# BayesLIM/BayesLIM

Hardware: AMD Instinct MI355X
Metric: visibilities/sec (Nbl x Ntime x Nfreq) fwd+bwd (higher is better)
Workload: dtype f32 (fringe sum: f16x3 split operands on the f16 MFMA -- 22-bit operands, f32 accumulate; phases f64); 1 GPU; HERA-128 (8128 bl), nside=128 diffuse + 1e4 point sources, 256 freqs; Nbl=8128, Nfreqs=256, Npix_sky=182664, Npix_visible=98304, Npoint=10000, beam=Airy D=14m on 1deg rect grid, linear PixelBeam interp, loss=sum |V|^2 (fused chi-square epilogue, rime_chisq_fwd / _bwd), parallelism=channel-sharded x1

## Files before the change

### bayeslim_amd/csrc/fringe_mfma.hip

```cpp
#include <hip/hip_runtime.h>
#include <hip/hip_fp16.h>
#include <type_traits>
#include "rime_common.h"

namespace rime {

typedef float f32x16 __attribute__((ext_vector_type(16)));
typedef _Float16 f16x8 __attribute__((ext_vector_type(8)));
typedef _Float16 f16x2 __attribute__((ext_vector_type(2)));

constexpr int MF_NA = 128;
constexpr int MF_SPLIT_PIX = 16384;

struct AntArgs {
    const double* antpos;
    const double* sdir;
    const double* freqs;
    const float* psky;
    const float* scale;
    const float* rowmin;
    const int* pair_direct;
    const int* pair_conj;
    float* vis;
    float* ws;
// ... 862 lines not shown
                if constexpr (!CEN) {
                    split2(w0 * c0, w1 * c1, rh, rl);
                    split2(w0 * s0, w1 * s1, ih, il);
                } else {
                    float xr0, xr1, xi0, xi1;
                    split2_prod(w0, c0, w1, c1, xr0, xr1, rh, rl);
                    split2_prod(w0, s0, w1, s1, xi0, xi1, ih, il);
                    cr[u] = fmaf(g0, xr0, cr[u]); keep_scalar(cr[u]); ci[u] = fmaf(g0, xi0, ci[u]);
                    cr[u] = fmaf(g1, xr1, cr[u]); keep_scalar(cr[u]); ci[u] = fmaf(g1, xi1, ci[u]);
                }
                unsigned char* o = buf + octet_row(u) * MF_ROWB + pp * 4 + 32 * hf;
                *reinterpret_cast<uint32_t*>(o) = rh;
                *reinterpret_cast<uint32_t*>(o + 2 * MF_KP) = ih;
                *reinterpret_cast<uint32_t*>(o + MF_IMG) = rl;
                *reinterpret_cast<uint32_t*>(o + MF_IMG + 2 * MF_KP) = il;
            }
        }
        fetch(next_panel);
    };

    const int foff = (lane & 31) * MF_ROWB + (lane >> 5) * 16;
    auto contract = [&](const unsigned char* buf) {
        auto frag = [&](int tile, int img, int im, int ks) {
            return *reinterpret_cast<const uint4*>(buf + img * MF_IMG + tile * 32 * MF_ROWB + foff + im * 2 * MF_KP + 32 * ks);
        };
        auto sgn = [&](uint4 v, const uint4& sg) {
            if constexpr (SIGNED) { v.x ^= sg.x; v.y ^= sg.y; v.z ^= sg.z; v.w ^= sg.w; }
            return v;
        };
#pragma unroll
        for (int ks = 0; ks < MF_NH; ++ks) {
            uint4 sg = make_uint4(0, 0, 0, 0);
            if constexpr (SIGNED) sg = *reinterpret_cast<const uint4*>(buf + 2 * MF_IMG + (2 * ks + (lane >> 5)) * 16);
            if constexpr (W == 0) {
                const uint4 Lrh = sgn(frag(0, 0, 0, ks), sg), Lih = sgn(frag(0, 0, 1, ks), sg);
                const uint4 Lrl = sgn(frag(0, 1, 0, ks), sg), Lil = sgn(frag(0, 1, 1, ks), sg);
                const uint4 Brh = frag(1, 0, 0, ks), Bih = frag(1, 0, 1, ks), Brl = frag(1, 1, 0, ks), Bil = frag(1, 1, 1, ks);
                acc[0] = RIME_MFMA(Lrh, Brh, acc[0]);
                acc[1] = RIME_MFMA(Lih, Bih, acc[1]);
                acc[0] = RIME_MFMA(Lrh, Brl, acc[0]);
                acc[1] = RIME_MFMA(Lih, Bil, acc[1]);
                acc[0] = RIME_MFMA(Lrl, Brh, acc[0]);
                acc[1] = RIME_MFMA(Lil, Bih, acc[1]);
            } else if constexpr (W == 1) {
                const uint4 Lrh = sgn(frag(0, 0, 0, ks), sg), Lih = sgn(frag(0, 0, 1, ks), sg);
                const uint4 Lrl = sgn(frag(0, 1, 0, ks), sg), Lil = sgn(frag(0, 1, 1, ks), sg);
                const uint4 Brh = frag(1, 0, 0, ks), Bih = frag(1, 0, 1, ks), Brl = frag(1, 1, 0, ks), Bil = frag(1, 1, 1, ks);
                acc[0] = RIME_MFMA(Lrh, Bih, acc[0]);
                acc[1] = RIME_MFMA(Lih, Brh, acc[1]);
                acc[0] = RIME_MFMA(Lrh, Bil, acc[0]);
                acc[1] = RIME_MFMA(Lih, Brl, acc[1]);
                acc[0] = RIME_MFMA(Lrl, Bih, acc[0]);
                acc[1] = RIME_MFMA(Lil, Brh, acc[1]);
            } else {
                constexpr int tt = W - 2;
                const uint4 Brh = frag(tt, 0, 0, ks), Bih = frag(tt, 0, 1, ks), Brl = frag(tt, 1, 0, ks), Bil = frag(tt, 1, 1, ks);
                const uint4 Lrh = sgn(Brh, sg), Lih = sgn(Bih, sg);
                const uint4 Hr = half_frag(Lrh), Hi = half_frag(Lih);
                acc[0] = RIME_MFMA(Hr, Brh, acc[0]);
                acc[1] = RIME_MFMA(Hi, Bih, acc[1]);
                acc[2] = RIME_MFMA(Lrh, Bih, acc[2]);
                acc[0] = RIME_MFMA(Lrh, Brl, acc[0]);
                acc[1] = RIME_MFMA(Lih, Bil, acc[1]);
                acc[3] = RIME_MFMA(Lih, Brl, acc[3]);
                acc[2] = RIME_MFMA(Lrh, Bil, acc[2]);
            }
        }
    };

    unsigned char* const buf0 = smem;
    unsigned char* const buf1 = smem + MF_BUF;
    fetch(pbeg);
    generate(buf0, min(pbeg + 1, pend - 1));
    __syncthreads();
    for (int panel = pbeg; panel < pend; panel += 2) {
        if (panel + 1 < pend) generate(buf1, min(panel + 2, pend - 1));
        contract(buf0);
        __syncthreads();
        if (panel + 1 < pend) {
            if (panel + 2 < pend) generate(buf0, min(panel + 3, pend - 1));
            contract(buf1);
        }
        __syncthreads();
    }

    float* dst = A.ws + (((size_t)split * A.Nt + t) * A.Nf + f) * 2 * A.Nbl;
    const float inv = 1.0f / scl;
    const int col = lane & 31, rb = 4 * (lane >> 5);
    RIME_MFMA_SETTLE();
    auto put = [&](int r, int c, float vr, float vi) {
        const int bd = A.pair_direct[r * MF_NA + c];
        if (bd >= 0) { dst[bd] = vr; dst[(size_t)A.Nbl + bd] = vi; }
        const int bc = A.pair_conj[r * MF_NA + c];
        if (bc >= 0) { dst[bc] = vr; dst[(size_t)A.Nbl + bc] = -vi; }
    };
    auto put1 = [&](int r, int c, int im, float v) {
        const int bd = A.pair_direct[r * MF_NA + c];
        if (bd >= 0) dst[(size_t)im * A.Nbl + bd] = v;
        const int bc = A.pair_conj[r * MF_NA + c];
        if (bc >= 0) dst[(size_t)im * A.Nbl + bc] = im ? -v : v;
    };
    if constexpr (CEN) {
#pragma unroll
        for (int u = 0; u < NGEN; ++u)
#pragma unroll
            for (int o = 1; o < 8; o <<= 1) { cr[u] += __shfl_xor(cr[u], o, 64); keep_scalar(cr[u]); ci[u] += __shfl_xor(ci[u], o, 64); keep_scalar(ci[u]); }
        float* cs = reinterpret_cast<float*>(smem) + 4 * (32 * 33);
        if (pp == 0) {
#pragma unroll
            for (int u = 0; u < NGEN; ++u)
                if (u < nk) { cs[(hf * 64 + octet_row(u)) * 2] = cr[u]; cs[(hf * 64 + octet_row(u)) * 2 + 1] = ci[u]; }
        }
        __syncthreads();
        if (tid < A.Nant) {
            float vr = cs[tid * 2] + cs[(64 + tid) * 2], vi = cs[tid * 2 + 1] + cs[(64 + tid) * 2 + 1];
            keep_scalar(vr); keep_scalar(vi);
            vr *= inv; keep_scalar(vr); vi *= inv;
            int b = A.centre[tid];
            if (b >= 0) { dst[b] = vr; dst[(size_t)A.Nbl + b] = vi; }
            b = A.centre[MF_NA + tid];
            if (b >= 0) { dst[b] = vr; dst[(size_t)A.Nbl + b] = -vi; }
            b = A.centre[64 + tid];
            if (b >= 0) { dst[b] = vr; dst[(size_t)A.Nbl + b] = -vi; }
            b = A.centre[MF_NA + 64 + tid];
            if (b >= 0) { dst[b] = vr; dst[(size_t)A.Nbl + b] = vi; }
        }
    }
    float* tr = reinterpret_cast<float*>(smem) + W * (32 * 33);
    auto transposed = [&](const f32x16& v) {
        f32x16 tv;
#pragma unroll
        for (int e = 0; e < 16; ++e) tr[((e & 3) + 8 * (e >> 2) + rb) * 33 + col] = v[e];
        asm volatile("s_waitcnt lgkmcnt(0)" ::: "memory");
#pragma unroll
        for (int e = 0; e < 16; ++e) tv[e] = tr[col * 33 + (e & 3) + 8 * (e >> 2) + rb];
        asm volatile("s_waitcnt lgkmcnt(0)" ::: "memory");
        return tv;
    };
    if constexpr (W < 2) {
        f32x16 s, d;
#pragma unroll
        for (int e = 0; e < 16; ++e) { s[e] = (acc[0][e] + acc[1][e]) * inv; d[e] = (acc[0][e] - acc[1][e]) * inv; }
        const f32x16 st = transposed(s), dt = transposed(d);
#pragma unroll
        for (int e = 0; e < 16; ++e) {
            const int re = (e & 3) + 8 * (e >> 2) + rb;
            const int i = re, j = 32 + col;
            const int it = col, jt = 32 + re;
            if constexpr (W == 0) {
                put1(i, j, 0, s[e]); put1(i, 64 + j, 0, d[e]);
                put1(64 + it, 64 + jt, 0, st[e]); put1(jt, 64 + it, 0, dt[e]);
            } else {
                put1(i, j, 1, d[e]); put1(i, 64 + j, 1, -s[e]);
                put1(64 + it, 64 + jt, 1, -dt[e]); put1(jt, 64 + it, 1, -st[e]);
            }
        }
    } else {
        constexpr int tt = W - 2;
        f32x16 ar, br, ai, bi, x, y;
#pragma unroll
        for (int e = 0; e < 16; ++e) { x[e] = acc[0][e] + acc[1][e]; y[e] = acc[0][e] - acc[1][e]; }
// ... 590 lines not shown
#pragma unroll
            for (int e = 0; e < 16; ++e) {
                const int an = 32 * ti + (e & 3) + 8 * (e >> 2) + 4 * h;
                const double ph = phase3(ant_lds[3 * an], sx, ant_lds[3 * an + 1], sy, ant_lds[3 * an + 2], sz);
                const float rr = turn_frac(ph);
                const float ce = __builtin_amdgcn_cosf(rr), se = __builtin_amdgcn_sinf(rr);
                part = fmaf(ce, accR[ti][e], part);
                part = fmaf(se, accI[ti][e], part);
                if constexpr (CPLX) {
                    pa = fmaf(se, accR[ti][e], pa);
                    pb = fmaf(ce, accI[ti][e], pb);
                }
                if ((e & 3) == 3) __builtin_amdgcn_sched_barrier(0);
            }
            if constexpr (CPLX) parti += pa - pb;
        }
        part += __shfl_xor(part, 32, 64);
        if constexpr (CPLX) parti += __shfl_xor(parti, 32, 64);
        if (h == 0) {
            float* o = orow + (size_t)p * A.st_p;
            if constexpr (CPLX) {
                const float im = parti * inv * A.imsign;
                float2* o2 = reinterpret_cast<float2*>(o);
                *o2 = A.accumulate ? make_float2(o2->x + part * inv, o2->y + im) : make_float2(part * inv, im);
            } else {
                *o = A.accumulate ? *o + part * inv : part * inv;
            }
        }
    }
}

struct PairBwdArgs : AntBwdArgs {
    const int* centre;
};

template <int TF> constexpr int pb_plane() { return (TF == 1 ? 1 : 3) * 2 * 2 * 32 * 16; }
constexpr int PB_THREADS = 256;
template <int TF> constexpr size_t pb_lds() { return 8 * (size_t)pb_plane<TF>() + 64 * 3 * sizeof(double) + 2 * 64 * sizeof(float); }

template <bool CEN, bool FLAT, int TF>
__global__ void __launch_bounds__(PB_THREADS, 3)
fringe_pair_bwd_kernel(PairBwdArgs A)
{
    constexpr int PB_PLANE = pb_plane<TF>();
    extern __shared__ __align__(16) unsigned char smem[];
    unsigned char* g_img = smem;
    double* ant_lds = reinterpret_cast<double*>(smem + 8 * PB_PLANE);
    float* cen_u = reinterpret_cast<float*>(smem + 8 * PB_PLANE + 64 * 3 * sizeof(double));
    float* cen_v = cen_u + 64;

    const int tid = threadIdx.x, lane = tid & 63, wave = __builtin_amdgcn_readfirstlane(tid >> 6);
    const int f = blockIdx.x % A.Nf, ts = blockIdx.x / A.Nf;
    const int t = ts / A.S, split = ts % A.S;
    const int TA = (A.Nant + 31) / 32;

    const double nu_c = A.sign * A.freqs[f] * (1.0 / 2.99792458e8);
    for (int i = tid; i < 64 * 3; i += PB_THREADS) ant_lds[i] = (i < A.Nant * 3) ? nu_c * A.antpos[i] : 0.0;
    const float gs = A.gscale[t * A.Nf + f] * 0.125f;
    const float* gre = A.gvt + ((size_t)t * A.Nf + f) * 2 * A.Nbl;
    const float* gim = gre + A.Nbl;
    auto grad_of = [&](int r, int c, float& vr, float& vi) {
        const int bd = A.pair_direct[r * MF_NA + c];
        if (bd >= 0) { vr += gre[bd]; keep_scalar(vr); vi += gim[bd]; keep_scalar(vi); }
        const int bc = A.pair_conj[r * MF_NA + c];
        if (bc >= 0) { vr += gre[bc]; keep_scalar(vr); vi -= gim[bc]; keep_scalar(vi); }
    };
    auto entry = [&](int i, int j, bool off, float& ar, float& ai, float& br, float& bi) {
        float xr = 0.f, xi = 0.f, yr = 0.f, yi = 0.f;
        grad_of(i, j, xr, xi);
        grad_of(64 + i, 64 + j, yr, yi);
        ar = xr + yr; keep_scalar(ar); ai = yi - xi;
        br = 0.f; bi = 0.f;
        grad_of(j, 64 + i, br, bi);
        if (off) grad_of(i, 64 + j, br, bi);
    };
    for (int e = tid; e < (TF == 1 ? 1 : 3) * 2 * 2 * 32 * 4; e += PB_THREADS) {
        const int jp = e & 3, row = (e >> 2) & 31, h = (e >> 7) & 1, ks = (e >> 8) & 1, tile = e >> 9;
        const int ti = tile == 2 ? 1 : 0, tj = tile == 0 ? 0 : 1;
        const int i = 32 * ti + row;
        const int j0 = 32 * tj + ((2 * jp) & 3) + 8 * (2 * ks + (jp >> 1)) + 4 * h;
        float n1[2] = {0.f, 0.f}, n2[2] = {0.f, 0.f}, n3[2] = {0.f, 0.f}, n4[2] = {0.f, 0.f};
        if (tj < TA) {
#pragma unroll
            for (int q = 0; q < 2; ++q) {
                const int j = j0 + q;
                float ar, ai, br, bi;
                entry(i, j, ti != tj, ar, ai, br, bi);
                if (ti != tj) {
                    n1[q] = ar + br; keep_scalar(n1[q]); n2[q] = ar - br; keep_scalar(n2[q]);
                    n3[q] = -(ai + bi); keep_scalar(n3[q]); n4[q] = ai - bi;
// ... 32 lines not shown
            b = A.centre[64 + tid];
            if (b >= 0) { u += gre[b]; keep_scalar(u); v -= gim[b]; keep_scalar(v); }
            b = A.centre[MF_NA + 64 + tid];
            if (b >= 0) { u += gre[b]; keep_scalar(u); v += gim[b]; keep_scalar(v); }
            u *= gs; keep_scalar(u); v *= gs;
            cen_u[tid] = u; cen_v[tid] = v;
        }
    }
    __syncthreads();

    const double* sd = A.sdir + (size_t)t * 3 * A.Pstride;
    float* orow = A.gpsky + (size_t)t * A.st_t + (size_t)f * A.st_f;
    const float inv = 1.0f / gs;
    const int h = lane >> 5;
    const int ntile = A.Pstride / 32;
    const int tbeg = split * A.tiles_per_split;
    const int tend = min(ntile, tbeg + A.tiles_per_split);

    const uint32_t gl0 = (h * 32 + (lane & 31)) * 16;
    for (int pt = tbeg + wave; pt < tend; pt += PB_THREADS / 64) {
        const int p = pt * 32 + (lane & 31);
        const double sx = sd[p], sy = sd[A.Pstride + p], sz = FLAT ? 0.0 : sd[2 * (size_t)A.Pstride + p];
        f32x16 accR[TF], accI[TF];
#pragma unroll
        for (int q = 0; q < TF; ++q)
#pragma unroll
            for (int e = 0; e < 16; ++e) {
                if constexpr (CEN) {
                    accR[q][e] = cen_u[32 * q + (e & 3) + 8 * (e >> 2) + 4 * h];
                    accI[q][e] = cen_v[32 * q + (e & 3) + 8 * (e >> 2) + 4 * h];
                } else { accR[q][e] = 0.f; accI[q][e] = 0.f; }
            }
        float part = 0.f;
#pragma unroll
        for (int tjr = 0; tjr < TF; ++tjr) {
            const int tj = TF - 1 - tjr;
            if (tj < TA) {
                float ec[16], es[16];
#pragma unroll
                for (int ks = 0; ks < 2; ++ks) {
                    if (32 * tj + 16 * ks >= A.Nant) {
#pragma unroll
                        for (int jj = 0; jj < 8; ++jj) { ec[8 * ks + jj] = 0.f; es[8 * ks + jj] = 0.f; }
                        continue;
                    }
                    uint4 Erh, Erl, Eih, Eil;
                    uint32_t* erh = reinterpret_cast<uint32_t*>(&Erh); uint32_t* erl = reinterpret_cast<uint32_t*>(&Erl);
                    uint32_t* eih = reinterpret_cast<uint32_t*>(&Eih); uint32_t* eil = reinterpret_cast<uint32_t*>(&Eil);
#pragma unroll
                    for (int jq = 0; jq < 2; ++jq) {
                        if (32 * tj + 16 * ks + 8 * jq >= A.Nant) {
#pragma unroll
                            for (int u = 0; u < 4; ++u) { ec[8 * ks + 4 * jq + u] = 0.f; es[8 * ks + 4 * jq + u] = 0.f; }
                            continue;
                        }
#pragma unroll
                        for (int u = 0; u < 4; ++u) {
                            const int jj = 4 * jq + u;
                            const int an = 32 * tj + (jj & 3) + 8 * (2 * ks + (jj >> 2)) + 4 * h;
                            const double ph = phase_of<FLAT>(ant_lds[3 * an], sx, ant_lds[3 * an + 1], sy, ant_lds[3 * an + 2], sz);
                            const float rr = turn_frac(ph);
                            ec[8 * ks + jj] = __builtin_amdgcn_cosf(rr);
                            es[8 * ks + jj] = __builtin_amdgcn_sinf(rr);
                        }
                    }
#pragma unroll
                    for (int q = 0; q < 4; ++q) {
                        split2_plain(ec[8 * ks + 2 * q], ec[8 * ks + 2 * q + 1], erh[q], erl[q]);
                        split2_plain(es[8 * ks + 2 * q], es[8 * ks + 2 * q + 1], eih[q], eil[q]);
                    }
#pragma unroll
                    for (int ti = 0; ti < TF; ++ti) {
                        if (ti <= tj) {
                            const int tk = ((ti + tj) * 2 + ks) * 1024;
                            const uint4 N1h = *reinterpret_cast<const uint4*>(g_img + gl0 + 0 * PB_PLANE + tk);
                            const uint4 N3h = *reinterpret_cast<const uint4*>(g_img + gl0 + 1 * PB_PLANE + tk);
                            const uint4 N2h = *reinterpret_cast<const uint4*>(g_img + gl0 + 2 * PB_PLANE + tk);
                            const uint4 N1l = *reinterpret_cast<const uint4*>(g_img + gl0 + 4 * PB_PLANE + tk);
                            const uint4 N3l = *reinterpret_cast<const uint4*>(g_img + gl0 + 5 * PB_PLANE + tk);
                            const uint4 N2l = *reinterpret_cast<const uint4*>(g_img + gl0 + 6 * PB_PLANE + tk);
                            if (ti == tj) {
                                accR[ti] = RIME_MFMA(N1h, Erh, accR[ti]);
                                accI[ti] = RIME_MFMA(N2h, Eih, accI[ti]);
                                accR[ti] = RIME_MFMA(N3h, Eih, accR[ti]);
                                accI[ti] = RIME_MFMA(N2h, Eil, accI[ti]);
                                accR[ti] = RIME_MFMA(N1h, Erl, accR[ti]);
// ... 173 lines not shown

}

using namespace rime;

static void ant_split_plan(int Nt, int Nf, int Pstride, int& S, int& panels_per_split)
{
    S = ant_splits(Nt, Nf, Pstride);
    const int npanel = Pstride / MF_KP;
    panels_per_split = (npanel + S - 1) / S;
    panels_per_split = ((panels_per_split + 3) / 4) * 4;
    S = (npanel + panels_per_split - 1) / panels_per_split;
}

extern "C" size_t rime_fringe_ant_workspace(int Nbl, int Nt, int Nf, int Pstride)
{
    int S, pps;
    ant_split_plan(Nt, Nf, Pstride, S, pps);
    return (size_t)S * Nbl * Nt * Nf * 2 * sizeof(float);
}

static bool fwd_packed_enabled()
{
    static const int on = [] { const char* e = getenv("RIME_FWD_PACKED"); return e ? atoi(e) : 1; }();
    return on != 0;
}

static bool bwd_small_enabled()
{
    static const int on = [] { const char* e = getenv("RIME_BWD_SMALL"); return e ? atoi(e) : 1; }();
    return on != 0;
}

static bool cross_shape_ok(int rows_i, int rows_j)
{
    return (rows_i == 32 && rows_j == 32) || (rows_i == 32 && rows_j == 64) || (rows_i == 64 && rows_j == 64) ||
           (rows_i == 128 && rows_j == 128);
}

static bool ant_common_ok(int Nrows, int cross, int Nbl, int Nt, int Nf, int Pstride, long long st_p, int sign, int cplx)
{
    if (st_p != 1 && st_p != 2) return false;
    if (cplx != 0 && (cplx != 1 && cplx != -1)) return false;
    if (cplx != 0 && st_p != 2) return false;
    if (cross && cross == Nrows) {
        if (cplx == 0 || !(Nrows == 32 || Nrows == 64 || Nrows == 96 || Nrows == 128)) return false;
    } else if (cross ? !cross_shape_ok(cross, Nrows - cross) : (Nrows <= 0 || Nrows > MF_NA)) return false;
    if (Nbl <= 0 || Nt <= 0 || Nt > 65535 || Nf <= 0 || Pstride <= 0 || Pstride % 64 != 0) return false;
    return sign == 1 || sign == -1;
}

template <int TI, int TJ>
static void launch_fwd_cross(const AntArgs& A, dim3 grid, hipStream_t st, bool has_rowmin, int cplx)
{
    using SH = FwdShape<TI, TJ, true>;
    if (cplx) {
        hipLaunchKernelGGL((fringe_ant_fwd_cross_kernel<TI, TJ, false, true>), grid, dim3(SH::NW * 64), SH::LDS, st, A);
        return;
    }
    hipLaunchKernelGGL((fringe_ant_fwd_cross_kernel<TI, TJ, true, false>), grid, dim3(SH::NW * 64), SH::LDS, st, A);
    if (has_rowmin) hipLaunchKernelGGL((fringe_ant_fwd_cross_kernel<TI, TJ, false, false>), grid, dim3(SH::NW * 64), SH::LDS, st, A);
}

extern "C" int rime_fringe_ant_fwd_block(const double* antpos, int Nrows, int cross, int mirror, const double* sdir,
                                         const double* freqs, const float* psky, const float* scale,
                                         const float* rowmin, const int* pair_direct, const int* pair_conj, int Nbl, int Nt, int Nf,
// ... 221 lines not shown
        } else {
            hipLaunchKernelGGL((fringe_pair_fwd1_kernel<true, false>), grid, dim3(256), lds1, st, A);
            if (rowmin) hipLaunchKernelGGL((fringe_pair_fwd1_kernel<false, false>), grid, dim3(256), lds1, st, A);
        }
        return check_launch();
    }
    using SH = FwdShape<2, 2, false>;
    static_assert(SH::LDS >= 4 * 33 * 32 * 4 + 2 * 64 * 2 * 4, "epilogue scratch: transposition tiles + the hub's column sums");
#define RIME_PAIR_FWD(CEN_, FLAT_)                                                                                       \
    do {                                                                                                                 \
        hipLaunchKernelGGL((fringe_pair_fwd_kernel<true, CEN_, FLAT_>), grid, dim3(256), SH::LDS, st, A);                \
        if (rowmin) hipLaunchKernelGGL((fringe_pair_fwd_kernel<false, CEN_, FLAT_>), grid, dim3(256), SH::LDS, st, A);   \
    } while (0)
    if (centre) { if (flat) RIME_PAIR_FWD(true, true); else RIME_PAIR_FWD(true, false); }
    else { if (flat) RIME_PAIR_FWD(false, true); else RIME_PAIR_FWD(false, false); }
#undef RIME_PAIR_FWD
    return check_launch();
}

extern "C" int rime_fringe_pair_bwd_block(const double* antpos, int Nrows, const int* centre, int flat, const double* sdir,
                                          const double* freqs, const float* gscale, const int* pair_direct,
                                          const int* pair_conj, int Nbl, int Nt, int Nf, int Pstride,
                                          long long st_t, long long st_f, long long st_p, int sign, int accumulate,
                                          float* gpsky, const void* workspace, size_t workspace_bytes, void* stream)
{
    if (!antpos || !sdir || !freqs || !gscale || !pair_direct || !pair_conj || !gpsky) return RIME_EINVAL;
    if (!pair_common_ok(Nrows, Nbl, Nt, Nf, Pstride, st_p, sign)) return RIME_EINVAL;
    if (!workspace || workspace_bytes < rime_fringe_ant_bwd_workspace(Nbl, Nt, Nf)) return RIME_EWORKSPACE;
    PairBwdArgs A{};
    A.antpos = antpos; A.sdir = sdir; A.freqs = freqs; A.gvis = nullptr; A.gscale = gscale;
    A.pair_direct = pair_direct; A.pair_conj = pair_conj; A.gpsky = gpsky; A.gvt = (const float*)workspace;
    A.Nant = Nrows; A.Nbl = Nbl; A.Nt = Nt; A.Nf = Nf; A.Pstride = Pstride;
    A.st_t = st_t; A.st_f = st_f; A.st_p = st_p; A.sign = (double)sign; A.accumulate = accumulate ? 1 : 0;
    A.rows_i = 0; A.imsign = 1.f; A.mirror = 0; A.centre = centre;
    const int ntile = Pstride / 32;
    int per = 256;
    while (per > 8 && (long)Nt * Nf * ((ntile + per - 1) / per) < 1024) per /= 2;
    A.tiles_per_split = per;
    A.S = (ntile + per - 1) / per;
    hipStream_t st = reinterpret_cast<hipStream_t>(stream);
    dim3 grid((unsigned)Nt * A.S * Nf, 1, 1);
    if (Nrows <= 32 && !centre) {
        if (flat) hipLaunchKernelGGL((fringe_pair_bwd_kernel<false, true, 1>), grid, dim3(PB_THREADS), pb_lds<1>(), st, A);
        else hipLaunchKernelGGL((fringe_pair_bwd_kernel<false, false, 1>), grid, dim3(PB_THREADS), pb_lds<1>(), st, A);
    } else if (centre) {
        if (flat) hipLaunchKernelGGL((fringe_pair_bwd_kernel<true, true, 2>), grid, dim3(PB_THREADS), pb_lds<2>(), st, A);
        else hipLaunchKernelGGL((fringe_pair_bwd_kernel<true, false, 2>), grid, dim3(PB_THREADS), pb_lds<2>(), st, A);
    } else {
        if (flat) hipLaunchKernelGGL((fringe_pair_bwd_kernel<false, true, 2>), grid, dim3(PB_THREADS), pb_lds<2>(), st, A);
        else hipLaunchKernelGGL((fringe_pair_bwd_kernel<false, false, 2>), grid, dim3(PB_THREADS), pb_lds<2>(), st, A);
    }
    return check_launch();
}
```

### bayeslim_amd/ops.py

```python
import ctypes
import os

import numpy as np
import torch

from . import _lib
from ._lib import lib, check, RIME_F32, RIME_F64

TILE = 64

PROFILE = None


def _require_cuda(*tensors):
    for t in tensors:
        if t is not None and not t.is_cuda:
            raise RuntimeError("bayeslim_amd ops need tensors on the GPU (got device '%s'); "
                               "there is no CPU implementation" % t.device)


def _stream():
    return ctypes.c_void_p(torch.cuda.current_stream().cuda_stream)


# ... 240 lines not shown
    if found is None:
        return None
    rows, mask, c = found
    newrow = -np.ones(n, dtype=np.int64)
    for r, a in enumerate(rows):
        if a >= 0:
            newrow[a] = r
    assert (newrow >= 0).all() and len(rows) <= 32 * ((n + 31) // 32)
    pos = np.zeros((len(rows), 3))
    for r, a in enumerate(rows):
        if a >= 0:
            pos[r] = P[a] - c
    direct = np.full((MFMA_GROUP, MFMA_GROUP), -1, dtype=np.int32)
    conj = np.full((MFMA_GROUP, MFMA_GROUP), -1, dtype=np.int32)
    od, oc = blk['direct'].reshape(MFMA_GROUP, MFMA_GROUP).cpu().numpy(), blk['conj'].reshape(MFMA_GROUP, MFMA_GROUP).cpu().numpy()
    for tab, swap in ((od, False), (oc, True)):
        for i, j in zip(*np.nonzero(tab >= 0)):
            a1, a2 = (j, i) if swap else (i, j)
            r1, r2 = newrow[a1], newrow[a2]
            if r1 // 32 <= r2 // 32:
                direct[r1, r2] = tab[i, j]
            else:
                conj[r2, r1] = tab[i, j]
    nd, nc = int((direct >= 0).sum()), int((conj >= 0).sum())
    assert nd + nc == int((od >= 0).sum()) + int((oc >= 0).sum())
    return dict(blk, pos=torch.as_tensor(pos, device=dev).contiguous(), nrows=len(rows), mirror=int(mask), rows=list(rows),
                cpass=(1 if nc == 0 else (-1 if nd == 0 else 0)), fwd_cpass=0, self_pos=None, mf_self=0,
                direct=torch.as_tensor(direct.reshape(-1), device=dev), conj=torch.as_tensor(conj.reshape(-1), device=dev))


PAIR = _env_int('RIME_PAIR', 1) != 0
PAIR_ROWS = 64
PAIR_CPLX = _env_int('RIME_PAIR_CPLX', 1) != 0


def _pair_layout(P, rows=PAIR_ROWS, hub_ok=True):
    found = _mirror_pairs(P)
    if found is None:
        return None
    c, pairs, singles = found
    hub = None
    if len(pairs) + len(singles) > rows:
        at_c = [a for a in singles if np.abs(np.asarray(P[a]) - c).max() <= MIRROR_TOL]
        if not hub_ok or not at_c or len(pairs) + len(singles) - 1 > rows:
            return None
        hub = at_c[0]
        singles = [a for a in singles if a != hub]
    firsts = [a for a, _ in pairs] + list(singles)
    partner = [b for _, b in pairs] + [-1] * len(singles)
    return firsts, partner, hub, c


def _pair_block(blk, P, dev):
    n = int(blk['nrows'])
    if blk['cross'] != 0 or n <= 32:
        return None
    lay = _pair_layout(P) if n > 64 else _pair_layout(P, rows=32, hub_ok=False)
    if lay is None:
        return None
    firsts, partner, hub, c = lay
    vrow = -np.ones(n, dtype=np.int64)
    for k, (a, b) in enumerate(zip(firsts, partner)):
        vrow[a] = k
        if b >= 0:
            vrow[b] = 64 + k
    direct = np.full((MFMA_GROUP, MFMA_GROUP), -1, dtype=np.int32)
    conj = np.full((MFMA_GROUP, MFMA_GROUP), -1, dtype=np.int32)
    centre = np.full((2, MFMA_GROUP), -1, dtype=np.int32)
    od, oc = blk['direct'].reshape(MFMA_GROUP, MFMA_GROUP).cpu().numpy(), blk['conj'].reshape(MFMA_GROUP, MFMA_GROUP).cpu().numpy()
    for tab, swap in ((od, False), (oc, True)):
        for i, j in zip(*np.nonzero(tab >= 0)):
            a1, a2 = (j, i) if swap else (i, j)
            if a1 == hub and a2 == hub:
                return None
            if a1 == hub:
                centre[0, vrow[a2]] = tab[i, j]
            elif a2 == hub:
                centre[1, vrow[a1]] = tab[i, j]
            else:
                r1, r2 = vrow[a1], vrow[a2]
                if r1 // 32 <= r2 // 32:
                    direct[r1, r2] = tab[i, j]
                else:
                    conj[r2, r1] = tab[i, j]
    nslots = int((direct >= 0).sum()) + int((conj >= 0).sum()) + int((centre >= 0).sum())
    assert nslots == int((od >= 0).sum()) + int((oc >= 0).sum())
    pos = np.asarray(P)[firsts] - c
    flat = int(np.abs(pos[:, 2]).max() <= MIRROR_TOL)
    if flat:
        pos[:, 2] = 0.0
    return dict(blk, pos=torch.as_tensor(pos, device=dev).contiguous(), nrows=len(firsts), mirror=0, pair=1,
                firsts=list(firsts), partner=list(partner), hub=hub, flat=flat,
                centre=None if hub is None else torch.as_tensor(centre.reshape(-1), device=dev),
                cpass=0, fwd_cpass=0, self_pos=None, mf_self=0, mf_fwd=26 if len(firsts) > 32 or hub is not None else 7,
                mf_bwd_real=30 if len(firsts) > 32 else 9,
                direct=torch.as_tensor(direct.reshape(-1), device=dev), conj=torch.as_tensor(conj.reshape(-1), device=dev))


def _dense_strides(t):
    if t.stride(-1) != 1:
        return None
    st = t.stride()
    P = t.shape[-1]
    if t.shape[3] > 1 and st[3] < P:
        return None
    if any(s <= 0 and n > 1 for s, n in zip(st[:4], t.shape[:4])):
        return None
    return (ctypes.c_longlong * 4)(*[int(max(s, 1)) for s in st[:4]])


def _pow2_scale(amax):
    safe = torch.where(amax > 0, amax, torch.ones_like(amax))
    e = torch.floor(torch.log2(16384.0 / safe)).clamp(-100.0, 100.0)
    return torch.where(amax > 0, torch.exp2(e), torch.ones_like(amax))


def _fringe_ant_call(geom, backward, inp, out, strides, Npp, cplx):
    a = geom.ant
    blocks = a.get('blocks_cplx', a['blocks']) if cplx else a.get('blocks_real', a['blocks'])
    tp_mask = a.get('two_pass_mask_cplx', a['two_pass_mask']) if cplx else a['two_pass_mask']
    m = 2 if cplx else 1
    st_t, st_mp, st_pp, st_f = (int(strides[k]) * m for k in range(4))
    Nbl, Nt, Nf, Nmp = geom.Nbl, geom.Nt, geom.Nf, geom.Nmp
    dev = inp.device
    geo = (_ptr(geom.sdir), _ptr(geom.freqs))
# ... 62 lines not shown
                for blk in two_pass:
                    flops += launch(blk, pp, 1, 0)
                check(lib.rime_fringe_ant_fwd_finish(_ptr(ws), ws.numel(), _ptr(tmp), Nbl, Nt, Nf, geom.Pstride,
                                                     _stream()), 'rime_fringe_ant_fwd_finish')
                if len(two_pass) < len(blocks):
                    tmp *= tp_mask
                out[pp][..., 0] -= tmp[..., 1]
                out[pp][..., 1] += tmp[..., 0]
    else:
        nbytes = lib.rime_fringe_ant_bwd_workspace(Nbl, Nt, Nf)
        ws = torch.empty(max(int(nbytes), 16), dtype=torch.uint8, device=dev)
        gvt = ws[:Nt * Nf * 2 * Nbl * 4].view(torch.float32).view(Nt * Nf, 2 * Nbl)
        two_pass = [blk for blk in blocks if cplx and blk['cpass'] == 0]
        for pp in range(Npp):
            written = set()
            for c in range(2 if two_pass else 1):
                g = inp[pp] if c == 0 else torch.stack([inp[pp][..., 1], -inp[pp][..., 0]], dim=-1).contiguous()
                check(lib.rime_fringe_ant_bwd_prepare(_ptr(g), Nbl, Nt, Nf, _ptr(ws), ws.numel(), _stream()),
                      'rime_fringe_ant_bwd_prepare')
                if c == 0:
                    scale_pp = torch.empty(Nt * Nf, dtype=torch.float32, device=dev)
                    check(lib.rime_fringe_row_scale(_ptr(gvt), 1, 1, 1, Nt * Nf, 0, 0, 0, 2 * Nbl, 2 * Nbl, _ptr(scale_pp),
                                                    None, _stream()), 'rime_fringe_row_scale')
                todo = sorted(blocks, key=lambda b: not (cplx and b['cpass'] != 0)) if c == 0 else two_pass
                for blk in todo:
                    single = cplx and blk['cpass'] != 0
                    mp = blk['mp']
                    planes = [(mp, 0), (mp, 1)] if single else [(mp, c)]
                    acc = int(planes[0] in written)
                    assert all((pl in written) == bool(acc) for pl in planes)
                    written.update(planes)
                    dst = ctypes.c_void_p(out.data_ptr() + 4 * (mp * st_mp + pp * st_pp + (0 if single else c)))
                    if blk.get('pair'):
                        rc = lib.rime_fringe_pair_bwd_block(_ptr(blk['pos']), blk['nrows'], _ptr(blk['centre']), blk['flat'], *geo,
                                                            _ptr(scale_pp), _ptr(blk['direct']), _ptr(blk['conj']),
                                                            *shape, acc, dst, _ptr(ws), ws.numel(), _stream())
                        check(rc, 'rime_fringe_pair_bwd_block')
                        flops += blk['mf_bwd_real']
                        continue
                    rc = lib.rime_fringe_ant_bwd_block(_ptr(blk['pos']), blk['nrows'], blk['cross'], blk['mirror'], *geo,
                                                       _ptr(scale_pp), _ptr(blk['direct']), _ptr(blk['conj']),
                                                       *shape, blk['cpass'] if single else 0, acc, dst,
                                                       _ptr(ws), ws.numel(), _stream())
                    check(rc, 'rime_fringe_ant_bwd_block')
                    flops += blk['mf_bwd'] if single else blk['mf_bwd_real']
            assert len(written) == Nmp * m, 'every psky plane must be written by a block'
    return flops * per16


def _setup_antenna_path(self, antpos, bl_ants, force=False, bl_mp=None, mp_pairs=None, group=MFMA_GROUP):
    Nant = int(antpos.shape[0])
    bl_ants = [(int(a), int(b)) for a, b in bl_ants]
    if Nant > MFMA_MAX_ANTS or len(bl_ants) != self.Nbl or self.Nt > 65535:
        return
    if not force and (Nant < MFMA_MIN_ANTS or self.Nbl < Nant * Nant // 8):
        return
    ant_model = None
    if bl_mp is not None and mp_pairs is not None and len(mp_pairs) > 1:
        ant_model = [None] * Nant
        for (a1, a2), mp in zip(bl_ants, bl_mp):
            for ant, mdl in ((a1, mp_pairs[mp][0]), (a2, mp_pairs[mp][1])):
                if ant_model[ant] is None:
                    ant_model[ant] = mdl
                elif ant_model[ant] != mdl:
                    return
        ant_model = [0 if mdl is None else mdl for mdl in ant_model]
    elif bl_mp is not None and any(int(x) != 0 for x in bl_mp):
        return
# ... 703 lines not shown
```

Measured before the change: 534.9 million vis/s.

## Share left-operand fragments across warp pair and exchange partial accumulators via LDS

```diff
diff --git a/bayeslim_amd/csrc/fringe_mfma.hip b/bayeslim_amd/csrc/fringe_mfma.hip
--- a/bayeslim_amd/csrc/fringe_mfma.hip
+++ b/bayeslim_amd/csrc/fringe_mfma.hip
@@ -918,26 +918,16 @@
         for (int ks = 0; ks < MF_NH; ++ks) {
             uint4 sg = make_uint4(0, 0, 0, 0);
             if constexpr (SIGNED) sg = *reinterpret_cast<const uint4*>(buf + 2 * MF_IMG + (2 * ks + (lane >> 5)) * 16);
-            if constexpr (W == 0) {
-                const uint4 Lrh = sgn(frag(0, 0, 0, ks), sg), Lih = sgn(frag(0, 0, 1, ks), sg);
-                const uint4 Lrl = sgn(frag(0, 1, 0, ks), sg), Lil = sgn(frag(0, 1, 1, ks), sg);
-                const uint4 Brh = frag(1, 0, 0, ks), Bih = frag(1, 0, 1, ks), Brl = frag(1, 1, 0, ks), Bil = frag(1, 1, 1, ks);
-                acc[0] = RIME_MFMA(Lrh, Brh, acc[0]);
-                acc[1] = RIME_MFMA(Lih, Bih, acc[1]);
-                acc[0] = RIME_MFMA(Lrh, Brl, acc[0]);
-                acc[1] = RIME_MFMA(Lih, Bil, acc[1]);
-                acc[0] = RIME_MFMA(Lrl, Brh, acc[0]);
-                acc[1] = RIME_MFMA(Lil, Bih, acc[1]);
-            } else if constexpr (W == 1) {
-                const uint4 Lrh = sgn(frag(0, 0, 0, ks), sg), Lih = sgn(frag(0, 0, 1, ks), sg);
-                const uint4 Lrl = sgn(frag(0, 1, 0, ks), sg), Lil = sgn(frag(0, 1, 1, ks), sg);
-                const uint4 Brh = frag(1, 0, 0, ks), Bih = frag(1, 0, 1, ks), Brl = frag(1, 1, 0, ks), Bil = frag(1, 1, 1, ks);
-                acc[0] = RIME_MFMA(Lrh, Bih, acc[0]);
-                acc[1] = RIME_MFMA(Lih, Brh, acc[1]);
-                acc[0] = RIME_MFMA(Lrh, Bil, acc[0]);
-                acc[1] = RIME_MFMA(Lih, Brl, acc[1]);
-                acc[0] = RIME_MFMA(Lrl, Bih, acc[0]);
-                acc[1] = RIME_MFMA(Lil, Brh, acc[1]);
+            if constexpr (W < 2) {
+                const uint4 Lh = sgn(frag(0, 0, W, ks), sg), Ll = sgn(frag(0, 1, W, ks), sg);
+                const uint4 Bsh = frag(1, 0, W, ks), Bsl = frag(1, 1, W, ks);
+                const uint4 Boh = frag(1, 0, 1 - W, ks), Bol = frag(1, 1, 1 - W, ks);
+                acc[0] = RIME_MFMA(Lh, Bsh, acc[0]);
+                acc[1] = RIME_MFMA(Lh, Boh, acc[1]);
+                acc[0] = RIME_MFMA(Lh, Bsl, acc[0]);
+                acc[1] = RIME_MFMA(Lh, Bol, acc[1]);
+                acc[0] = RIME_MFMA(Ll, Bsh, acc[0]);
+                acc[1] = RIME_MFMA(Ll, Boh, acc[1]);
             } else {
                 constexpr int tt = W - 2;
                 const uint4 Brh = frag(tt, 0, 0, ks), Bih = frag(tt, 0, 1, ks), Brl = frag(tt, 1, 0, ks), Bil = frag(tt, 1, 1, ks);
@@ -974,6 +964,12 @@
     const float inv = 1.0f / scl;
     const int col = lane & 31, rb = 4 * (lane >> 5);
     RIME_MFMA_SETTLE();
+    if constexpr (W < 2) {
+        float* xo = reinterpret_cast<float*>(smem) + (1 - W) * (32 * 33);
+#pragma unroll
+        for (int e = 0; e < 16; ++e) xo[e * 64 + lane] = acc[1 - W][e];
+    }
+    if constexpr (!CEN) __syncthreads();
     auto put = [&](int r, int c, float vr, float vi) {
         const int bd = A.pair_direct[r * MF_NA + c];
         if (bd >= 0) { dst[bd] = vr; dst[(size_t)A.Nbl + bd] = vi; }
@@ -1013,6 +1009,11 @@
         }
     }
     float* tr = reinterpret_cast<float*>(smem) + W * (32 * 33);
+    if constexpr (W < 2) {
+#pragma unroll
+        for (int e = 0; e < 16; ++e) acc[1 - W][e] = tr[e * 64 + lane];
+        asm volatile("s_waitcnt lgkmcnt(0)" ::: "memory");
+    }
     auto transposed = [&](const f32x16& v) {
         f32x16 tv;
 #pragma unroll
```

Measured after the change: 540.9 million vis/s (median of 6 runs). 1.01x the previous value.

## Reuse arithmetic-progression antenna phases via rotation in pair backward kernel

Applied to the files above, without the earlier changes.

```diff
diff --git a/bayeslim_amd/csrc/fringe_mfma.hip b/bayeslim_amd/csrc/fringe_mfma.hip
--- a/bayeslim_amd/csrc/fringe_mfma.hip
+++ b/bayeslim_amd/csrc/fringe_mfma.hip
@@ -1669,7 +1669,17 @@
 
 struct PairBwdArgs : AntBwdArgs {
     const int* centre;
+    int ap;
 };
+
+__device__ __forceinline__ void rotate_scalar(float c, float s, float dc, float ds, float& oc, float& os)
+{
+    float t = c * dc; keep_scalar(t);
+    oc = fmaf(-s, ds, t); keep_scalar(oc);
+    float w = s * dc; keep_scalar(w);
+    os = fmaf(c, ds, w); keep_scalar(os);
+}
+constexpr double PAIR_AP_TOL = 1e-9;
 
 template <int TF> constexpr int pb_plane() { return (TF == 1 ? 1 : 3) * 2 * 2 * 32 * 16; }
 constexpr int PB_THREADS = 256;
@@ -1693,6 +1703,24 @@
 
     const double nu_c = A.sign * A.freqs[f] * (1.0 / 2.99792458e8);
     for (int i = tid; i < 64 * 3; i += PB_THREADS) ant_lds[i] = (i < A.Nant * 3) ? nu_c * A.antpos[i] : 0.0;
+    uint32_t apmask = 0;
+    double dnx = 0.0, dny = 0.0, dnz = 0.0;
+    if (A.ap && A.Nant >= 8) {
+        const double dx = A.antpos[3] - A.antpos[0], dy = A.antpos[4] - A.antpos[1], dz = A.antpos[5] - A.antpos[2];
+        bool ok = false;
+        if (lane < 8 && 8 * lane + 8 <= A.Nant) {
+            ok = true;
+            for (int q = 8 * lane; q < 8 * lane + 8; q += 4)
+                for (int k = 1; k < 4; ++k) {
+                    const double* r0 = A.antpos + 3 * q;
+                    const double* rk = r0 + 3 * k;
+                    ok = ok && fabs(rk[0] - r0[0] - k * dx) <= PAIR_AP_TOL && fabs(rk[1] - r0[1] - k * dy) <= PAIR_AP_TOL
+                            && fabs(rk[2] - r0[2] - k * dz) <= PAIR_AP_TOL;
+                }
+        }
+        apmask = __builtin_amdgcn_readfirstlane((uint32_t)__ballot(ok)) & 0xffu;
+        dnx = nu_c * dx; dny = nu_c * dy; dnz = nu_c * dz;
+    }
     const float gs = A.gscale[t * A.Nf + f] * 0.125f;
     const float* gre = A.gvt + ((size_t)t * A.Nf + f) * 2 * A.Nbl;
     const float* gim = gre + A.Nbl;
@@ -1791,6 +1819,11 @@
                 } else { accR[q][e] = 0.f; accI[q][e] = 0.f; }
             }
         float part = 0.f;
+        float Dc = 1.f, Ds = 0.f;
+        if (apmask) {
+            const float rr = turn_frac(phase_of<FLAT>(dnx, sx, dny, sy, dnz, sz));
+            Dc = __builtin_amdgcn_cosf(rr); Ds = __builtin_amdgcn_sinf(rr);
+        }
 #pragma unroll
         for (int tjr = 0; tjr < TF; ++tjr) {
             const int tj = TF - 1 - tjr;
@@ -1811,6 +1844,19 @@
                         if (32 * tj + 16 * ks + 8 * jq >= A.Nant) {
 #pragma unroll
                             for (int u = 0; u < 4; ++u) { ec[8 * ks + 4 * jq + u] = 0.f; es[8 * ks + 4 * jq + u] = 0.f; }
+                            continue;
+                        }
+                        if ((apmask >> (4 * tj + 2 * ks + jq)) & 1u) {
+                            const int an = 32 * tj + 8 * (2 * ks + jq) + 4 * h + 1;
+                            const double ph = phase_of<FLAT>(ant_lds[3 * an], sx, ant_lds[3 * an + 1], sy, ant_lds[3 * an + 2], sz);
+                            const float rr = turn_frac(ph);
+                            float* c4 = ec + 8 * ks + 4 * jq;
+                            float* s4 = es + 8 * ks + 4 * jq;
+                            c4[1] = __builtin_amdgcn_cosf(rr);
+                            s4[1] = __builtin_amdgcn_sinf(rr);
+                            rotate_scalar(c4[1], s4[1], Dc, -Ds, c4[0], s4[0]);
+                            rotate_scalar(c4[1], s4[1], Dc, Ds, c4[2], s4[2]);
+                            rotate_scalar(c4[2], s4[2], Dc, Ds, c4[3], s4[3]);
                             continue;
                         }
 #pragma unroll
@@ -2050,6 +2096,12 @@
     return on != 0;
 }
 
+static bool pair_ap_enabled()
+{
+    static const int on = [] { const char* e = getenv("RIME_PAIR_AP"); return e ? atoi(e) : 1; }();
+    return on != 0;
+}
+
 static bool cross_shape_ok(int rows_i, int rows_j)
 {
     return (rows_i == 32 && rows_j == 32) || (rows_i == 32 && rows_j == 64) || (rows_i == 64 && rows_j == 64) ||
@@ -2337,7 +2389,7 @@
     A.pair_direct = pair_direct; A.pair_conj = pair_conj; A.gpsky = gpsky; A.gvt = (const float*)workspace;
     A.Nant = Nrows; A.Nbl = Nbl; A.Nt = Nt; A.Nf = Nf; A.Pstride = Pstride;
     A.st_t = st_t; A.st_f = st_f; A.st_p = st_p; A.sign = (double)sign; A.accumulate = accumulate ? 1 : 0;
-    A.rows_i = 0; A.imsign = 1.f; A.mirror = 0; A.centre = centre;
+    A.rows_i = 0; A.imsign = 1.f; A.mirror = 0; A.centre = centre; A.ap = pair_ap_enabled() ? 1 : 0;
     const int ntile = Pstride / 32;
     int per = 256;
     while (per > 8 && (long)Nt * Nf * ((ntile + per - 1) / per) < 1024) per /= 2;
diff --git a/bayeslim_amd/ops.py b/bayeslim_amd/ops.py
--- a/bayeslim_amd/ops.py
+++ b/bayeslim_amd/ops.py
@@ -296,9 +296,10 @@
 PAIR = _env_int('RIME_PAIR', 1) != 0
 PAIR_ROWS = 64
 PAIR_CPLX = _env_int('RIME_PAIR_CPLX', 1) != 0
-
-
-def _pair_layout(P, rows=PAIR_ROWS, hub_ok=True):
+PAIR_AP = _env_int('RIME_PAIR_AP', 1) != 0
+
+
+def _pair_layout(P, rows=PAIR_ROWS, hub_ok=True, ap=False):
     found = _mirror_pairs(P)
     if found is None:
         return None
@@ -312,7 +313,71 @@
         singles = [a for a in singles if a != hub]
     firsts = [a for a, _ in pairs] + list(singles)
     partner = [b for _, b in pairs] + [-1] * len(singles)
+    if ap:
+        order = _pair_ap_order(np.asarray(P, dtype=np.float64)[firsts] - c)
+        firsts, partner = [firsts[k] for k in order], [partner[k] for k in order]
     return firsts, partner, hub, c
+
+
+def _pair_ap_mask(pos):
+    pos = np.asarray(pos, dtype=np.float64)
+    n = len(pos)
+    if n < 8:
+        return 0
+    d = pos[1] - pos[0]
+    mask = 0
+    for m in range(n // 8):
+        ok = all(np.abs(pos[q + k] - pos[q] - k * d).max() <= MIRROR_TOL for q in (8 * m, 8 * m + 4) for k in (1, 2, 3))
+        mask |= int(ok) << m
+    return mask
+
+
+def _pair_ap_order(pos):
+    pos = np.asarray(pos, dtype=np.float64)
+    n = len(pos)
+    ident = list(range(n))
+    if n < 8:
+        return ident
+    diff = pos[None, :, :] - pos[:, None, :]
+    length = np.sqrt((diff ** 2).sum(-1))
+    length[np.arange(n), np.arange(n)] = np.inf
+    short = length.min()
+    if not np.isfinite(short) or short <= MIRROR_TOL:
+        return ident
+    cands = []
+    for a, b in zip(*np.nonzero(length <= short * (1 + 1e-6))):
+        d = diff[a, b]
+        if not any(np.abs(d - e).max() <= MIRROR_TOL or np.abs(d + e).max() <= MIRROR_TOL for e in cands):
+            cands.append(d)
+    best = []
+    for d in cands:
+        succ = -np.ones(n, dtype=np.int64)
+        for a in range(n):
+            hit = np.nonzero(np.abs(diff[a] - d).max(-1) <= MIRROR_TOL)[0]
+            if len(hit):
+                succ[a] = hit[0]
+        has_pred = set(succ[succ >= 0].tolist())
+        quads = []
+        for a in range(n):
+            if a in has_pred:
+                continue
+            line = [a]
+            while succ[line[-1]] >= 0 and succ[line[-1]] not in line:
+                line.append(int(succ[line[-1]]))
+            quads += [line[4 * q:4 * q + 4] for q in range(len(line) // 4)]
+        if quads:
+            step = pos[quads[0][1]] - pos[quads[0][0]]
+            quads = [q for q in quads if all(np.abs(pos[q[k]] - pos[q[0]] - k * step).max() <= MIRROR_TOL for k in (1, 2, 3))]
+        if len(quads) > len(best):
+            best = quads
+    noct = len(best) // 2
+    if noct == 0:
+        return ident
+    lead = [a for q in best[:2 * noct] for a in q]
+    taken = set(lead)
+    order = lead + [a for a in ident if a not in taken]
+    assert sorted(order) == ident
+    return order
 
 
 def _pair_block(blk, P, dev):
@@ -323,38 +388,56 @@
     if lay is None:
         return None
     firsts, partner, hub, c = lay
-    vrow = -np.ones(n, dtype=np.int64)
-    for k, (a, b) in enumerate(zip(firsts, partner)):
-        vrow[a] = k
-        if b >= 0:
-            vrow[b] = 64 + k
-    direct = np.full((MFMA_GROUP, MFMA_GROUP), -1, dtype=np.int32)
-    conj = np.full((MFMA_GROUP, MFMA_GROUP), -1, dtype=np.int32)
-    centre = np.full((2, MFMA_GROUP), -1, dtype=np.int32)
     od, oc = blk['direct'].reshape(MFMA_GROUP, MFMA_GROUP).cpu().numpy(), blk['conj'].reshape(MFMA_GROUP, MFMA_GROUP).cpu().numpy()
-    for tab, swap in ((od, False), (oc, True)):
-        for i, j in zip(*np.nonzero(tab >= 0)):
-            a1, a2 = (j, i) if swap else (i, j)
-            if a1 == hub and a2 == hub:
-                return None
-            if a1 == hub:
-                centre[0, vrow[a2]] = tab[i, j]
-            elif a2 == hub:
-                centre[1, vrow[a1]] = tab[i, j]
-            else:
-                r1, r2 = vrow[a1], vrow[a2]
-                if r1 // 32 <= r2 // 32:
-                    direct[r1, r2] = tab[i, j]
+
+    def tables(firsts, partner):
+        vrow = -np.ones(n, dtype=np.int64)
+        for k, (a, b) in enumerate(zip(firsts, partner)):
+            vrow[a] = k
+            if b >= 0:
+                vrow[b] = 64 + k
+        direct = np.full((MFMA_GROUP, MFMA_GROUP), -1, dtype=np.int32)
+        conj = np.full((MFMA_GROUP, MFMA_GROUP), -1, dtype=np.int32)
+        centre = np.full((2, MFMA_GROUP), -1, dtype=np.int32)
+        for tab, swap in ((od, False), (oc, True)):
+            for i, j in zip(*np.nonzero(tab >= 0)):
+                a1, a2 = (j, i) if swap else (i, j)
+                if a1 == hub and a2 == hub:
+                    return None
+                if a1 == hub:
+                    centre[0, vrow[a2]] = tab[i, j]
+                elif a2 == hub:
+                    centre[1, vrow[a1]] = tab[i, j]
                 else:
-                    conj[r2, r1] = tab[i, j]
-    nslots = int((direct >= 0).sum()) + int((conj >= 0).sum()) + int((centre >= 0).sum())
-    assert nslots == int((od >= 0).sum()) + int((oc >= 0).sum())
+                    r1, r2 = vrow[a1], vrow[a2]
+                    if r1 // 32 <= r2 // 32:
+                        direct[r1, r2] = tab[i, j]
+                    else:
+                        conj[r2, r1] = tab[i, j]
+        nslots = int((direct >= 0).sum()) + int((conj >= 0).sum()) + int((centre >= 0).sum())
+        assert nslots == int((od >= 0).sum()) + int((oc >= 0).sum())
+        slots = np.sort(np.concatenate([t[t >= 0] for t in (direct, conj, centre)]))
+        assert np.array_equal(slots, np.sort(np.concatenate([od[od >= 0], oc[oc >= 0]]))) and (np.diff(slots) > 0).all()
+        return direct, conj, centre
+
+    tabs = tables(firsts, partner)
+    if tabs is None:
+        return None
+    direct, conj, centre = tabs
     pos = np.asarray(P)[firsts] - c
     flat = int(np.abs(pos[:, 2]).max() <= MIRROR_TOL)
     if flat:
         pos[:, 2] = 0.0
+    dev_t = lambda x: torch.as_tensor(x, device=dev).contiguous()
+    bwd = None
+    order = _pair_ap_order(pos) if PAIR_AP else list(range(len(firsts)))
+    if order != list(range(len(firsts))):
+        bf, bp = [firsts[k] for k in order], [partner[k] for k in order]
+        bd, bc, bcen = tables(bf, bp)
+        bwd = dict(firsts=bf, partner=bp, pos=dev_t(pos[order]), direct=dev_t(bd.reshape(-1)), conj=dev_t(bc.reshape(-1)),
+                   centre=None if hub is None else dev_t(bcen.reshape(-1)))
     return dict(blk, pos=torch.as_tensor(pos, device=dev).contiguous(), nrows=len(firsts), mirror=0, pair=1,
-                firsts=list(firsts), partner=list(partner), hub=hub, flat=flat,
+                firsts=list(firsts), partner=list(partner), hub=hub, flat=flat, bwd=bwd,
                 centre=None if hub is None else torch.as_tensor(centre.reshape(-1), device=dev),
                 cpass=0, fwd_cpass=0, self_pos=None, mf_self=0, mf_fwd=26 if len(firsts) > 32 or hub is not None else 7,
                 mf_bwd_real=30 if len(firsts) > 32 else 9,
@@ -483,8 +566,9 @@
                     written.update(planes)
                     dst = ctypes.c_void_p(out.data_ptr() + 4 * (mp * st_mp + pp * st_pp + (0 if single else c)))
                     if blk.get('pair'):
-                        rc = lib.rime_fringe_pair_bwd_block(_ptr(blk['pos']), blk['nrows'], _ptr(blk['centre']), blk['flat'], *geo,
-                                                            _ptr(scale_pp), _ptr(blk['direct']), _ptr(blk['conj']),
+                        rows = blk.get('bwd') or blk
+                        rc = lib.rime_fringe_pair_bwd_block(_ptr(rows['pos']), blk['nrows'], _ptr(rows['centre']), blk['flat'], *geo,
+                                                            _ptr(scale_pp), _ptr(rows['direct']), _ptr(rows['conj']),
                                                             *shape, acc, dst, _ptr(ws), ws.numel(), _stream())
                         check(rc, 'rime_fringe_pair_bwd_block')
                         flops += blk['mf_bwd_real']
```

New measurement: 526.1 million vis/s before, 537.7 million vis/s after, median of 6. +2.2%, better.
